# berkeley-hipie/HIPIE

Measured on AMD Instinct MI355X. Metric: images/sec @1024x1024 ViT-H bs=8 (single-image inference hot path: box, class and mask logits), higher is better.
Workload: dtype f16x3 (split-fp16 operands, fp32 accumulate: fp32-class); 1 GPU; BASELINE.json configs[2]: vit_huge, 1024x1024, batch 8 per GPU, 80 class prompts (L=194), detection; global_batch=8, parallelism=dp1, precision_policy=split, launch=eager

## Files before the change

hipie_amd/csrc/gemm.hip:

```cpp
#include "gemm_tile.h"

namespace hipie {

template <typename T>
__global__ __launch_bounds__(256) void to_hl8_kernel(const T* __restrict__ x, f16_t* __restrict__ out, long rows, int K, long ldx, long ldo,
                                                     float scale) {
  const long gid = (long)blockIdx.x * 256 + threadIdx.x;
  const int gpr = K / 8;
  if (gid >= rows * gpr) return;
  const long r = gid / gpr;
  const int g = (int)(gid - r * gpr);
  const T* src = x + r * ldx + 8 * g;
  f16x8 h, l;
#pragma unroll
  for (int e = 0; e < 8; ++e) {
    f16_t hh, ll;
    hl_split((float)src[e] * scale, hh, ll);
    h[e] = hh;
    l[e] = ll;
  }
  f16_t* dst = out + r * ldo + 16 * g;
  *reinterpret_cast<f16x8*>(dst) = h;
  *reinterpret_cast<f16x8*>(dst + 8) = l;
}


constexpr int kTrRows = 128, kTrCols = 64;
__global__ __launch_bounds__(256) void to_hl8_t_kernel(const float* __restrict__ x, f16_t* __restrict__ out, long rows, int C, long ldx,
                                                       long ldo, long rows_p, float scale) {
  __shared__ float tile[kTrRows][kTrCols + 1];
  const long r0 = (long)blockIdx.x * kTrRows;
  const int c0 = blockIdx.y * kTrCols;
  const int tid = threadIdx.x;
  for (int k = tid; k < kTrRows * (kTrCols / 4); k += 256) {
    const int i = k / (kTrCols / 4), j = (k % (kTrCols / 4)) * 4;
    float v[4] = {0.f, 0.f, 0.f, 0.f};
    if (r0 + i < rows) {
      const float* src = x + (r0 + i) * ldx + c0 + j;
      if (c0 + j + 3 < C && (((uintptr_t)src) & 15) == 0) {
        const float4 q = *reinterpret_cast<const float4*>(src);
        v[0] = q.x; v[1] = q.y; v[2] = q.z; v[3] = q.w;
      } else {
        for (int e = 0; e < 4; ++e) v[e] = c0 + j + e < C ? src[e] : 0.f;
      }
    }
    for (int e = 0; e < 4; ++e) tile[i][j + e] = v[e];
  }
  __syncthreads();
  for (int u = tid; u < kTrCols * (kTrRows / 8); u += 256) {
    const int g = u % (kTrRows / 8), c = u / (kTrRows / 8);
    const long m = r0 + 8 * g;
    if (c0 + c >= C || m >= rows_p) continue;
    f16x8 h, l;
#pragma unroll
    for (int e = 0; e < 8; ++e) {
      f16_t hh, ll;
      hl_split(tile[8 * g + e][c] * scale, hh, ll);
      h[e] = hh;
      l[e] = ll;
    }
    f16_t* dst = out + (long)(c0 + c) * ldo + 2 * m;
    *reinterpret_cast<f16x8*>(dst) = h;
    *reinterpret_cast<f16x8*>(dst + 8) = l;
  }
}

}

using namespace hipie;

namespace hipie {
int launch_gemm_k256(const void* X, long ldx_b, int x_f32, const void* W, long ldw_b, const float* bias, float* out, long ldo, int M, int N,
                     hipStream_t st);
}

static inline bool gemm_mfma16() {
  const char* e = study_env("HIPIE_GEMM_MFMA");
  return e ? atoi(e) == 16 : true;
}

static int gemm_impl(const void* A, int64_t lda, const void* W, int64_t ldw, const float* bias, const float* resid, int64_t ldr,
                     void* out, int64_t ldo, const int32_t* out_row, const int32_t* a_row, int64_t a_rows, int M, int N, int K, int in_fmt,
                     int out_fmt, int act, float alpha, float oscale, void* stream, const float* alpha_dev = nullptr) {
  HIPIE_REQUIRE(A && W && out, "gemm: null pointer");
  HIPIE_REQUIRE(in_fmt == HIPIE_F16 || in_fmt == HIPIE_HL8 || in_fmt == HIPIE_F32, "gemm: operand format %d (HIPIE_F16 | HIPIE_HL8 | HIPIE_F32)",
                in_fmt);
  HIPIE_REQUIRE(out_fmt == HIPIE_F32 || out_fmt == HIPIE_F16 || out_fmt == HIPIE_HL8, "gemm: output format %d", out_fmt);
  HIPIE_REQUIRE(act >= 0 && act <= 3, "gemm: activation %d (0 none, 1 gelu, 2 relu, 3 quick-gelu)", act);
  HIPIE_REQUIRE(M > 0 && N > 0 && K > 0 && N % 8 == 0, "gemm: M=%d N=%d K=%d (N must be a multiple of 8)", M, N, K);
  const bool a_f32 = in_fmt == HIPIE_F32;
  const bool split = in_fmt == HIPIE_HL8 || a_f32;
  if (a_f32) lda *= 2;
  const int kq = split ? 32 : 64;
  HIPIE_REQUIRE(K % kq == 0, "gemm: K=%d must be a multiple of %d", K, kq);
  const int epr = split ? 2 * K : K;
  HIPIE_TRY(gm_check_operands("gemm", lda, ldw, epr, 320));
  HIPIE_TRY(gm_check_out("gemm", ldo, out_fmt, N));
  HIPIE_TRY(gm_check_resid("gemm", resid, ldr, N));
  HIPIE_TRY(gm_check_aligned("gemm", {A, W, out, bias, resid}));
  GemmParams p;
  gm_set_operands(p, A, lda, W, ldw, M, N, K, kq);
  p.bias = bias; p.resid = resid; p.ldr = ldr; p.out = (char*)out; p.ldo = ldo; p.out_row = out_row; p.a_row = a_row;
  p.out_fmt = out_fmt; p.act = act; p.alpha = alpha; p.oscale = oscale; p.alpha_dev = alpha_dev;
  hipStream_t st = (hipStream_t)stream;
  static const int k256_mode = [] { const char* e = study_env("HIPIE_GEMM_K256"); return e ? atoi(e) : 2; }();
  const bool k256_on = k256_mode == 1 || (k256_mode == 2 && N >= 384);
  if (k256_on && split && K == 256 && out_fmt == HIPIE_F32 && act == 0 && resid == nullptr && out_row == nullptr && a_row == nullptr &&
      alpha == 1.f && oscale == 1.f && alpha_dev == nullptr && N % 32 == 0 && M >= 8192 && ldw * 2 == 1024 && (long)M * p.lda_b < (1L << 32))
    return launch_gemm_k256(A, p.lda_b, a_f32 ? 1 : 0, W, p.ldw_b, bias, (float*)out, ldo, M, N, st);
  const bool wide = (N % 320 == 0);
  static const int small_on = [] { const char* e = study_env("HIPIE_GEMM_SMALL"); return e ? atoi(e) : 1; }();
  static const long small_tiles = [] { const char* e = study_env("HIPIE_GEMM_SMALL_MAXTILES"); return e ? atol(e) : 96L; }();
  const bool small_ok = small_on && (long)((M + 255) / 256) * ((N + (wide ? 319 : 255)) / (wide ? 320 : 256)) < small_tiles;
#ifdef HIPIE_GEMM_VARIANTS
  { const char* e = study_env("HIPIE_GEMM_VARIANT"); const int v = e ? atoi(e) : 0;
    if (split && wide && v == 1) return launch_gemm<320, true, 1>(p, st);
    if (split && wide && v == 3) return launch_gemm<320, true, 3>(p, st); }
  { const char* e = study_env("HIPIE_GEMM_VARIANT"); if (e) p.variant = atoi(e); }
  p.prio_mode = gemm2_prio();
  if (split && gemm2_mode() == 4) {
    const bool w160 = (N % 160 == 0);
    if (a_f32) return w160 ? launch_gemm4<5, 2>(p, st) : launch_gemm4<4, 2>(p, st);
    return w160 ? launch_gemm4<5, 0>(p, st) : launch_gemm4<4, 0>(p, st);
  }
  if (split && gemm2_mode() == 2) {
    const bool w160 = (N % 160 == 0);
    if (a_f32) return w160 ? launch_gemm3<5, 2>(p, st) : launch_gemm3<4, 2>(p, st);
    return w160 ? launch_gemm3<5, 0>(p, st) : launch_gemm3<4, 0>(p, st);
  }
  if (split && gemm2_mode() == 1) {
    const bool w160 = (N % 160 == 0);
    if (a_f32) return w160 ? launch_gemm2<5, 2>(p, st) : launch_gemm2<4, 2>(p, st);
    return w160 ? launch_gemm2<5, 0>(p, st) : launch_gemm2<4, 0>(p, st);
  }
#endif
  if (split && small_ok && a_row == nullptr) return a_f32 ? launch_gemm_small<2>(p, st) : launch_gemm_small<0>(p, st);
  if (split && wide && gemm_mfma16()) return a_f32 ? launch_gemm<320, true, 2, 16>(p, st) : launch_gemm<320, true, 0, 16>(p, st);
  if (a_f32) return wide ? launch_gemm<320, true, 2>(p, st) : launch_gemm<256, true, 2>(p, st);
  if (split) return wide ? launch_gemm<320, true>(p, st) : launch_gemm<256, true>(p, st);
  return wide ? launch_gemm<320, false>(p, st) : launch_gemm<256, false>(p, st);
}

extern "C" int hipie_gemm(const void* A, int64_t lda, const void* W, int64_t ldw, const float* bias, const float* resid, int64_t ldr,
                          void* out, int64_t ldo, const int32_t* out_row, int M, int N, int K, int in_fmt, int out_fmt, int act, float alpha,
                          float oscale, void* stream) {
  return gemm_impl(A, lda, W, ldw, bias, resid, ldr, out, ldo, out_row, nullptr, 0, M, N, K, in_fmt, out_fmt, act, alpha, oscale, stream);
}

extern "C" int hipie_gemm_scaled(const void* A, int64_t lda, const void* W, int64_t ldw, const float* bias, const float* resid, int64_t ldr,
                                 void* out, int64_t ldo, const int32_t* out_row, int M, int N, int K, int in_fmt, int out_fmt, int act, float alpha,
                                 float oscale, const float* alpha_dev, void* stream) {
  HIPIE_REQUIRE(((uintptr_t)alpha_dev % 4) == 0, "gemm_scaled: alpha_dev must be 4-byte aligned");
  return gemm_impl(A, lda, W, ldw, bias, resid, ldr, out, ldo, out_row, nullptr, 0, M, N, K, in_fmt, out_fmt, act, alpha, oscale, stream, alpha_dev);
}

extern "C" int hipie_gemm_gather(const void* A, int64_t lda, int64_t a_rows, const int32_t* a_row, const void* W, int64_t ldw, const float* bias,
                                 const float* resid, int64_t ldr, void* out, int64_t ldo, const int32_t* out_row, int M, int N, int K, int in_fmt,
                                 int out_fmt, int act, float alpha, float oscale, void* stream) {
  HIPIE_REQUIRE(a_row != nullptr && a_rows > 0, "gemm_gather: a_row map / operand row count missing");
  HIPIE_REQUIRE(in_fmt == HIPIE_HL8 || in_fmt == HIPIE_F32, "gemm_gather: split operands only (HIPIE_HL8 | HIPIE_F32 rows)");
  HIPIE_REQUIRE((long)a_rows * lda * (in_fmt == HIPIE_F32 ? 4 : 2) < (1L << 32), "gemm_gather: the gathered operand must stay below 4 GiB");
  return gemm_impl(A, lda, W, ldw, bias, resid, ldr, out, ldo, out_row, a_row, a_rows, M, N, K, in_fmt, out_fmt, act, alpha, oscale, stream);
}

extern "C" int hipie_gemm_batched(const void* A, int64_t lda, int64_t a_outer, int64_t a_inner, const void* W, int64_t ldw, int64_t w_outer,
                                  int64_t w_inner, void* out, int64_t ldo, int64_t o_outer, int64_t o_inner, int n_outer, int n_inner, int M,
                                  int N, int K, int out_fmt, float alpha, void* stream) {
  HIPIE_REQUIRE(A && W && out, "gemm_batched: null pointer");
  HIPIE_REQUIRE(out_fmt == HIPIE_F32 || out_fmt == HIPIE_HL8, "gemm_batched: output format %d (HIPIE_F32 | HIPIE_HL8)", out_fmt);
  HIPIE_REQUIRE(M > 0 && N > 0 && K > 0 && N % 8 == 0 && K % 32 == 0, "gemm_batched: M=%d N=%d K=%d (N %% 8, K %% 32)", M, N, K);
  HIPIE_TRY(gm_check_batch_shape("gemm_batched", n_outer, n_inner));
  HIPIE_TRY(gm_check_operands("gemm_batched", lda, ldw, 2 * K, 320));
  HIPIE_TRY(gm_check_out("gemm_batched", ldo, out_fmt, N));
  HIPIE_TRY(gm_check_batch_offsets("gemm_batched", a_outer, a_inner, w_outer, w_inner, o_outer, o_inner));
  HIPIE_TRY(gm_check_aligned("gemm_batched", {A, W, out}));
  GemmParams p;
  gm_set_operands(p, A, lda, W, ldw, M, N, K);
  gm_set_batch(p, n_inner, a_outer, a_inner, w_outer, w_inner, o_outer, o_inner, out_fmt == HIPIE_F32 ? 4 : 2);
  p.out = (char*)out; p.ldo = ldo; p.out_fmt = out_fmt; p.alpha = alpha;
  hipStream_t st = (hipStream_t)stream;
  const int batches = n_outer * n_inner;
#ifdef HIPIE_GEMM_VARIANTS
  if (gemm2_mode() == 1) return (N % 160 == 0) ? launch_gemm2<5, 0>(p, st, batches) : launch_gemm2<4, 0>(p, st, batches);
#endif
  return (N % 320 == 0) ? launch_gemm<320, true>(p, st, batches) : launch_gemm<256, true>(p, st, batches);
}

extern "C" int hipie_gemm_batched_resid(const void* A, int64_t lda, int64_t a_outer, int64_t a_inner, const void* W, int64_t ldw, int64_t w_outer,
                                        int64_t w_inner, const float* bias, const float* resid, int64_t ldr, int64_t r_outer, int64_t r_inner,
                                        float* out, int64_t ldo, int64_t o_outer, int64_t o_inner, int n_outer, int n_inner, int M, int N, int K,
                                        float alpha, void* stream) {
  HIPIE_REQUIRE(A && W && out, "gemm_batched_resid: null pointer");
  HIPIE_REQUIRE(M > 0 && N > 0 && K > 0 && N % 8 == 0 && K % 32 == 0, "gemm_batched_resid: M=%d N=%d K=%d (N %% 8, K %% 32)", M, N, K);
  HIPIE_TRY(gm_check_batch_shape("gemm_batched_resid", n_outer, n_inner));
  HIPIE_TRY(gm_check_operands("gemm_batched_resid", lda, ldw, 2 * K, 320));
  HIPIE_TRY(gm_check_out("gemm_batched_resid", ldo, HIPIE_F32, N));
  HIPIE_REQUIRE(resid == nullptr || (ldr >= N && ldr % 4 == 0 && ((r_outer | r_inner) % 4) == 0), "gemm_batched_resid: residual strides %ld / %ld / %ld",
                (long)ldr, (long)r_outer, (long)r_inner);
  HIPIE_TRY(gm_check_batch_offsets("gemm_batched_resid", a_outer, a_inner, w_outer, w_inner, o_outer, o_inner));
  HIPIE_TRY(gm_check_aligned("gemm_batched_resid", {A, W, out, bias, resid}));
  GemmParams p;
  gm_set_operands(p, A, lda, W, ldw, M, N, K);
  gm_set_batch(p, n_inner, a_outer, a_inner, w_outer, w_inner, o_outer, o_inner, 4);
  p.out = (char*)out; p.ldo = ldo; p.alpha = alpha;
  p.bias = bias; p.resid = resid; p.ldr = ldr; p.r_bo = r_outer; p.r_bi = r_inner;
  return (N % 320 == 0) ? launch_gemm<320, true>(p, (hipStream_t)stream, n_outer * n_inner) : launch_gemm<256, true>(p, (hipStream_t)stream, n_outer * n_inner);
}

extern "C" int hipie_gemm_batched_softmax(const void* A, int64_t lda, int64_t a_outer, int64_t a_inner, const void* W, int64_t ldw, int64_t w_outer,
                                          int64_t w_inner, void* out, int64_t ldo, int64_t o_outer, int64_t o_inner, int n_outer, int n_inner,
                                          int M, int N, int K, const unsigned char* mask, int L, float clamp, float alpha, void* stream) {
  HIPIE_REQUIRE(A && W && out, "gemm_batched_softmax: null pointer");
  HIPIE_REQUIRE(M > 0 && N > 0 && N <= 256 && N % 8 == 0 && K > 0 && K % 32 == 0 && L > 0 && L <= N,
                "gemm_batched_softmax: M=%d N=%d K=%d L=%d (N <= 256: the row must fit one column tile)", M, N, K, L);
  HIPIE_TRY(gm_check_batch_shape("gemm_batched_softmax", n_outer, n_inner));
  HIPIE_TRY(gm_check_operands("gemm_batched_softmax", lda, ldw, 2 * K, 320));
  HIPIE_TRY(gm_check_out("gemm_batched_softmax", ldo, HIPIE_HL8, N));
  HIPIE_TRY(gm_check_batch_offsets("gemm_batched_softmax", a_outer, a_inner, w_outer, w_inner, o_outer, o_inner));
  HIPIE_TRY(gm_check_aligned("gemm_batched_softmax", {A, W, out}));
  GemmParams p;
  gm_set_operands(p, A, lda, W, ldw, M, N, K);
  gm_set_batch(p, n_inner, a_outer, a_inner, w_outer, w_inner, o_outer, o_inner, 2);
  p.out = (char*)out; p.ldo = ldo; p.out_fmt = HIPIE_HL8; p.alpha = alpha;
  p.softmax = 1; p.sm_L = L; p.sm_clamp = clamp; p.sm_mask = mask;
  return launch_gemm<256, true>(p, (hipStream_t)stream, n_outer * n_inner);
}

extern "C" int hipie_conv3x3_split(const void* x, int64_t ldx, const void* w, const float* bias, void* out, int64_t ldo, int64_t rows, int Wp,
                                   int C, int N, int in_fmt, int out_fmt, int act, void* stream) {
  HIPIE_REQUIRE(x && w && out, "conv3x3_split: null pointer");
  HIPIE_REQUIRE(in_fmt == HIPIE_HL8 || in_fmt == HIPIE_F32, "conv3x3_split: input format %d (HIPIE_HL8 | HIPIE_F32 rows)", in_fmt);
  HIPIE_REQUIRE(out_fmt == HIPIE_F32 || out_fmt == HIPIE_HL8, "conv3x3_split: output format %d (HIPIE_F32 | HIPIE_HL8)", out_fmt);
  HIPIE_REQUIRE(act >= 0 && act <= 2, "conv3x3_split: activation %d", act);
  HIPIE_REQUIRE(rows > 0 && rows < (1L << 31) && Wp >= 3 && C > 0 && C % 32 == 0 && N > 0 && N % 8 == 0, "conv3x3_split: rows=%ld Wp=%d C=%d N=%d",
                (long)rows, Wp, C, N);
  if (in_fmt == HIPIE_F32) ldx *= 2;
  HIPIE_REQUIRE(ldx >= 2 * C && ldx % 8 == 0, "conv3x3_split: input row stride %ld", (long)ldx);
  HIPIE_REQUIRE((long)(256 + Wp + 2) * ldx * 2 < (1L << 31), "conv3x3_split: row stride too large");
  HIPIE_TRY(gm_check_out("conv3x3_split", ldo, out_fmt, N));
  HIPIE_TRY(gm_check_aligned("conv3x3_split", {x, w, out, bias}));
  GemmParams p;
  gm_set_operands(p, x, ldx, w, (long)2 * 9 * C, (int)rows, N, 9 * C);
  p.bias = bias; p.out = (char*)out; p.ldo = ldo; p.out_fmt = out_fmt; p.act = act;
  p.conv_kpt = C / 32; p.conv_wp = Wp;
  hipStream_t st = (hipStream_t)stream;
  const bool wide = (N % 320 == 0);
  if (in_fmt == HIPIE_F32) return wide ? launch_gemm<320, true, 2>(p, st) : launch_gemm<256, true, 2>(p, st);
  return wide ? launch_gemm<320, true>(p, st) : launch_gemm<256, true>(p, st);
}

extern "C" int hipie_to_hl8(const void* x, int64_t ldx, void* out, int64_t ldo, int64_t rows, int K, int x_dtype, float scale, void* stream) {
  HIPIE_REQUIRE(x && out && rows > 0 && K > 0 && K % 8 == 0, "to_hl8: rows=%ld K=%d (K must be a multiple of 8)", (long)rows, K);
  HIPIE_REQUIRE(ldx >= K && ldo >= 2 * K && ldo % 8 == 0, "to_hl8: row strides %ld / %ld", (long)ldx, (long)ldo);
  const long n = rows * (K / 8);
  const dim3 grid((unsigned)((n + 255) / 256));
  hipStream_t st = (hipStream_t)stream;
  switch (x_dtype) {
    case HIPIE_F32: hipLaunchKernelGGL(to_hl8_kernel<float>, grid, dim3(256), 0, st, (const float*)x, (f16_t*)out, rows, K, ldx, ldo, scale); break;
    case HIPIE_F16: hipLaunchKernelGGL(to_hl8_kernel<f16_t>, grid, dim3(256), 0, st, (const f16_t*)x, (f16_t*)out, rows, K, ldx, ldo, scale); break;
    default: return set_err(HIPIE_EINVAL, "to_hl8: dtype %d", x_dtype);
  }
  return check_launch("to_hl8");
}

extern "C" int hipie_to_hl8_t(const void* x, int64_t ldx, void* out, int64_t ldo, int64_t rows, int C, int64_t rows_p, float scale, void* stream) {
  HIPIE_REQUIRE(x && out && rows > 0 && C > 0, "to_hl8_t: rows=%ld C=%d", (long)rows, C);
  HIPIE_REQUIRE(rows_p >= rows && rows_p % 8 == 0 && ldx >= C && ldo >= 2 * rows_p && ldo % 8 == 0, "to_hl8_t: rows_p=%ld (>= rows, multiple of 8), strides %ld / %ld",
                (long)rows_p, (long)ldx, (long)ldo);
  HIPIE_REQUIRE(((uintptr_t)out % 16) == 0, "to_hl8_t: output must be 16-byte aligned");
  const long tiles_r = (rows_p + kTrRows - 1) / kTrRows, tiles_c = (C + kTrCols - 1) / kTrCols;
  HIPIE_REQUIRE(tiles_c <= 65535, "to_hl8_t: C=%d too wide", C);
  hipLaunchKernelGGL(to_hl8_t_kernel, dim3((unsigned)tiles_r, (unsigned)tiles_c), dim3(256), 0, (hipStream_t)stream, (const float*)x, (f16_t*)out,
                     (long)rows, C, (long)ldx, (long)ldo, (long)rows_p, scale);
  return check_launch("to_hl8_t");
}
```

hipie_amd/csrc/layernorm.hip:

```cpp
#include "common.h"
#include "row_norm.h"

namespace hipie {

struct hl8_t { unsigned int u; };
template <> struct Vec4<hl8_t> {
  static __device__ __forceinline__ void load(const hl8_t* p, float (&v)[4]) {
    const char* q = reinterpret_cast<const char*>(p);
    const bool second = (reinterpret_cast<uintptr_t>(q) & 16) != 0;
    const f16x4 h = *reinterpret_cast<const f16x4*>(second ? q - 8 : q);
    const f16x4 l = *reinterpret_cast<const f16x4*>(second ? q + 8 : q + 16);
#pragma unroll
    for (int i = 0; i < 4; ++i) v[i] = (float)h[i] + (float)l[i];
  }
  static __device__ __forceinline__ void store(hl8_t* p, const float (&v)[4]) {
    char* q = reinterpret_cast<char*>(p);
    const bool second = (reinterpret_cast<uintptr_t>(q) & 16) != 0;
    f16x4 h, l;
#pragma unroll
    for (int i = 0; i < 4; ++i) {
      f16_t hh, ll;
      hl_split(v[i], hh, ll);
      h[i] = hh;
      l[i] = ll;
    }
    *reinterpret_cast<f16x4*>(second ? q - 8 : q) = h;
    *reinterpret_cast<f16x4*>(second ? q + 8 : q + 16) = l;
  }
};

template <typename Tx, typename Td, typename Tn>
__global__ __launch_bounds__(256) void add_layernorm_kernel(const Tx* __restrict__ x, const Td* __restrict__ delta,
                                                            const float* __restrict__ gamma, const float* __restrict__ beta,
                                                            Tx* __restrict__ res_out, Tn* __restrict__ norm_out, long rows,
                                                            int C, float eps, const int32_t* __restrict__ delta_row,
                                                            const int32_t* __restrict__ out_src, const Tn* __restrict__ addend,
                                                            Tn* __restrict__ sum_out) {
  const long orow = (long)blockIdx.x * 4 + (threadIdx.x >> 6);
  if (orow >= rows) return;
  const LnRow r(C);
  const long row = out_src ? (long)out_src[orow] : orow;
  if (row < 0) {
    const float z[4] = {0.f, 0.f, 0.f, 0.f};
    for (int i = 0; i <= r.nv; ++i)
      if ((i < r.nv)|| (r.lane < r.tail)) Vec4<Tn>::store(norm_out + orow * C + r.col(i), z);
    return;
  }
  const long drow = delta_row ? (long)delta_row[row] : row;
  float v[LN_MAXV][4];
  float sum = 0.f;
  const Tx* xr = x + row * C;
#pragma unroll
  for (int i = 0; i < LN_MAXV; ++i) {
    if (r.on(i)) {
      const int c = r.col(i);
      Vec4<Tx>::load(xr + c, v[i]);
      if (delta != nullptr) {
        float d[4];
        Vec4<Td>::load(delta + drow * C + c, d);
#pragma unroll
        for (int e = 0; e < 4; ++e) v[i][e] += d[e];
      }
      if (res_out != nullptr) Vec4<Tx>::store(res_out + row * C + c, v[i]);
#pragma unroll
      for (int e = 0; e < 4; ++e) sum += v[i][e];
    } else {
#pragma unroll
      for (int e = 0; e < 4; ++e) v[i][e] = 0.f;
    }
  }
  sum = wave_sum(sum);
  const float mean = sum / (float)C;
  float sq = 0.f;
#pragma unroll
  for (int i = 0; i < LN_MAXV; ++i) {
    if (r.on(i)) {
#pragma unroll
      for (int e = 0; e < 4; ++e) { const float d = v[i][e] - mean; sq += d * d; }
    }
  }
  sq = wave_sum(sq);
  const float rstd = rsqrtf(sq / (float)C + eps);
#pragma unroll
  for (int i = 0; i < LN_MAXV; ++i) {
    if (r.on(i)) {
      const int c = r.col(i);
      float o[4];
      ln_affine(v[i], mean, rstd, gamma + c, beta + c, o);
      Vec4<Tn>::store(norm_out + orow * C + c, o);
      if (sum_out != nullptr) {
        float a[4];
        Vec4<Tn>::load(addend + orow * C + c, a);
#pragma unroll
        for (int e = 0; e < 4; ++e) a[e] += o[e];
        Vec4<Tn>::store(sum_out + orow * C + c, a);
      }
    }
  }
}

struct LnArgs {
  const void* x; const void* delta; const float* gamma; const float* beta; void* res_out; void* norm_out;
  long rows; int C; float eps;
  int x_dtype, delta_dtype, norm_dtype;
  hipStream_t stream;
  const int32_t* delta_row = nullptr; const int32_t* out_src = nullptr;
  const void* addend = nullptr; void* sum_out = nullptr;
};

template <typename Tx, typename Td, typename Tn>
static int launch_ln(const LnArgs& a) {
  hipLaunchKernelGGL((add_layernorm_kernel<Tx, Td, Tn>), dim3((unsigned)((a.rows + 3) / 4)), dim3(256), 0, a.stream, (const Tx*)a.x,
                     (const Td*)a.delta, a.gamma, a.beta, (Tx*)a.res_out, (Tn*)a.norm_out, a.rows, a.C, a.eps, a.delta_row, a.out_src,
                     (const Tn*)a.addend, (Tn*)a.sum_out);
  return check_launch("add_layernorm");
}

static int add_layernorm(const LnArgs& a) {
  HIPIE_REQUIRE(a.x && a.gamma && a.beta && a.norm_out, "add_layernorm: null pointer");
  HIPIE_REQUIRE(a.rows >= 0 && a.C > 0 && a.C % 4 == 0 && a.C <= LN_MAXV * 256, "add_layernorm: C=%d must be a multiple of 4 and <= %d", a.C, LN_MAXV * 256);
  if (a.rows == 0) return HIPIE_OK;
  return with_dtype(a.x_dtype, "add_layernorm: bad x dtype", [&](auto tx) {
    return with_dtype(a.delta_dtype, "add_layernorm: bad delta dtype", [&](auto td) {
      using Tx = decltype(tx);
      using Td = decltype(td);
      if (a.norm_dtype == HIPIE_HL8) {
        if (a.C % 8 != 0 || (reinterpret_cast<uintptr_t>(a.norm_out) & 31) != 0) return set_err(HIPIE_EINVAL, "add_layernorm: HL8 output needs C %% 8 == 0 and a 32-byte aligned buffer");
        return launch_ln<Tx, Td, hl8_t>(a);
      }
      return with_dtype(a.norm_dtype, "add_layernorm: bad norm dtype", [&](auto tn) { return launch_ln<Tx, Td, decltype(tn)>(a); });
    });
  });
}


template <typename Td, typename Ta>
__global__ __launch_bounds__(256) void add_layernorm_dec_kernel(const float* __restrict__ x, const Td* __restrict__ delta,
                                                                const float* __restrict__ gamma, const float* __restrict__ beta,
                                                                float* __restrict__ norm_out, Ta* __restrict__ norm16,
                                                                const Ta* __restrict__ addend, Ta* __restrict__ sum16, long rows,
                                                                int C, float eps) {
  const long row = (long)blockIdx.x * 4 + (threadIdx.x >> 6);
  if (row >= rows) return;
  const LnRow r(C);
  float v[LN_MAXV][4];
  float sum = 0.f;
#pragma unroll
  for (int i = 0; i < LN_MAXV; ++i) {
    if (r.on(i)) {
      const long c = row * C + r.col(i);
      float d[4];
      Vec4<float>::load(x + c, v[i]);
      Vec4<Td>::load(delta + c, d);
#pragma unroll
      for (int e = 0; e < 4; ++e) { v[i][e] += d[e]; sum += v[i][e]; }
    } else {
#pragma unroll
      for (int e = 0; e < 4; ++e) v[i][e] = 0.f;
    }
  }
  float mean, rstd;
  ln_row_stats(r, v, sum, C, eps, mean, rstd);
#pragma unroll
  for (int i = 0; i < LN_MAXV; ++i) {
    if (r.on(i)) {
      const int cc = r.col(i);
      const long c = row * C + cc;
      float o[4];
      ln_affine(v[i], mean, rstd, gamma + cc, beta + cc, o);
      Vec4<float>::store(norm_out + c, o);
      if (norm16 != nullptr) Vec4<Ta>::store(norm16 + c, o);
      if (sum16 != nullptr) {
        float a[4];
        Vec4<Ta>::load(addend + c, a);
#pragma unroll
        for (int e = 0; e < 4; ++e) a[e] += o[e];
        Vec4<Ta>::store(sum16 + c, a);
      }
    }
  }
}

template <typename Td, typename Ta>
static int launch_ln_dec(const float* x, const void* d, const float* g, const float* b, float* n, void* n16, const void* add,
                         void* s16, long rows, int C, float eps, hipStream_t st) {
  hipLaunchKernelGGL((add_layernorm_dec_kernel<Td, Ta>), dim3((unsigned)((rows + 3) / 4)), dim3(256), 0, st, x, (const Td*)d, g, b,
                     n, (Ta*)n16, (const Ta*)add, (Ta*)s16, rows, C, eps);
  return check_launch("add_layernorm_dec");
}

template <typename Ta>
__global__ __launch_bounds__(256) void add_cast_kernel(const float* __restrict__ a, const Ta* __restrict__ b, Ta* __restrict__ out, long n4) {
  const long i = (long)blockIdx.x * 256 + threadIdx.x;
  if (i >= n4) return;
  float x[4], y[4];
  Vec4<float>::load(a + 4 * i, x);
  Vec4<Ta>::load(b + 4 * i, y);
#pragma unroll
  for (int e = 0; e < 4; ++e) x[e] += y[e];
  Vec4<Ta>::store(out + 4 * i, x);
}

}

extern "C" int hipie_add_layernorm(const void* x, const void* delta, const float* gamma, const float* beta, void* res_out,
                                   void* norm_out, int64_t rows, int C, float eps, int x_dtype, int delta_dtype,
                                   int norm_dtype, void* stream) {
  return hipie::add_layernorm({x, delta, gamma, beta, res_out, norm_out, rows, C, eps, x_dtype, delta_dtype, norm_dtype, (hipStream_t)stream});
}

extern "C" int hipie_add_layernorm_rows(const void* x, const void* delta, const float* gamma, const float* beta,
                                        void* res_out, void* norm_out, int64_t out_rows, int C, float eps, int x_dtype,
                                        int delta_dtype, int norm_dtype, const int32_t* delta_row, const int32_t* out_src,
                                        void* stream) {
  hipie::LnArgs a = {x, delta, gamma, beta, res_out, norm_out, out_rows, C, eps, x_dtype, delta_dtype, norm_dtype, (hipStream_t)stream};
  a.delta_row = delta_row;
  a.out_src = out_src;
  return hipie::add_layernorm(a);
}

extern "C" int hipie_add_layernorm_dec(const float* x, const void* delta, const float* gamma, const float* beta, float* norm_out,
                                       void* norm16_out, const void* addend, void* sum16_out, int64_t rows, int C, float eps,
                                       int delta_dtype, int aux_dtype, void* stream) {
  using namespace hipie;
  HIPIE_REQUIRE(x && delta && gamma && beta && norm_out, "add_layernorm_dec: null pointer");
  HIPIE_REQUIRE((sum16_out == nullptr) || (addend != nullptr), "add_layernorm_dec: sum16_out needs addend");
  HIPIE_REQUIRE(rows >= 0 && C > 0 && C % 4 == 0 && C <= LN_MAXV * 256, "add_layernorm_dec: C=%d must be a multiple of 4 and <= %d", C, LN_MAXV * 256);
  HIPIE_REQUIRE(aux_dtype == HIPIE_F16 || aux_dtype == HIPIE_BF16 || aux_dtype == HIPIE_HL8, "add_layernorm_dec: aux dtype must be f16, bf16 or HL8");
  HIPIE_REQUIRE(aux_dtype != HIPIE_HL8 || (C % 8 == 0 && (((uintptr_t)norm16_out | (uintptr_t)addend | (uintptr_t)sum16_out) & 31) == 0),
                "add_layernorm_dec: HL8 outputs need C %% 8 == 0 and 32-byte aligned buffers");
  if (rows == 0) return HIPIE_OK;
  hipStream_t st = (hipStream_t)stream;
  return with_dtype(delta_dtype, "add_layernorm_dec: bad delta dtype", [&](auto td) {
    auto launch = [&](auto ta) {
      return launch_ln_dec<decltype(td), decltype(ta)>(x, delta, gamma, beta, norm_out, norm16_out, addend, sum16_out, rows, C, eps, st);
    };
    return aux_dtype == HIPIE_F16 ? launch(f16_t()) : aux_dtype == HIPIE_HL8 ? launch(hl8_t()) : launch(bf16_t());
  });
}

extern "C" int hipie_add_cast(const float* a, const void* b, void* out, int64_t n, int dtype, void* stream) {
  using namespace hipie;
  HIPIE_REQUIRE(a && b && out, "add_cast: null pointer");
  HIPIE_REQUIRE(n >= 0 && n % 4 == 0, "add_cast: n must be a multiple of 4");
  HIPIE_REQUIRE(dtype == HIPIE_F16 || dtype == HIPIE_BF16 || dtype == HIPIE_HL8, "add_cast: dtype must be f16, bf16 or HL8");
  HIPIE_REQUIRE(dtype != HIPIE_HL8 || (n % 8 == 0 && (((uintptr_t)b | (uintptr_t)out) & 31) == 0), "add_cast: HL8 needs n %% 8 == 0 and 32-byte aligned buffers");
  if (n == 0) return HIPIE_OK;
  hipStream_t st = (hipStream_t)stream;
  const long n4 = n / 4;
  const unsigned grid = (unsigned)((n4 + 255) / 256);
  auto launch = [&](auto t) {
    using Ta = decltype(t);
    hipLaunchKernelGGL((add_cast_kernel<Ta>), dim3(grid), dim3(256), 0, st, a, (const Ta*)b, (Ta*)out, n4);
  };
  if (dtype == HIPIE_HL8) launch(hl8_t());
  else if (dtype == HIPIE_F16) launch(f16_t());
  else launch(bf16_t());
  return check_launch("add_cast");
}

extern "C" int hipie_add_layernorm_sum(const void* x, const void* delta, const float* gamma, const float* beta, void* res_out,
                                       void* norm_out, const void* addend, void* sum_out, int64_t rows, int C, float eps,
                                       int x_dtype, int delta_dtype, int norm_dtype, void* stream) {
  using namespace hipie;
  HIPIE_REQUIRE((addend == nullptr) == (sum_out == nullptr), "add_layernorm_sum: addend and sum_out go together");
  LnArgs a = {x, delta, gamma, beta, res_out, norm_out, rows, C, eps, x_dtype, delta_dtype, norm_dtype, (hipStream_t)stream};
  a.addend = addend;
  a.sum_out = sum_out;
  return add_layernorm(a);
}
```

hipie_amd/modeling/vit.py:

```python
import math

import torch
import torch.nn as nn
import torch.nn.functional as F

from .. import ops
from ..derived import derived, stamp


def get_rel_pos(q_size, k_size, rel_pos):
    max_rel_dist = int(2 * max(q_size, k_size) - 1)
    if rel_pos.shape[0] != max_rel_dist:
        r = F.interpolate(rel_pos.reshape(1, rel_pos.shape[0], -1).permute(0, 2, 1), size=max_rel_dist, mode="linear")
        r = r.reshape(-1, max_rel_dist).permute(1, 0)
    else:
        r = rel_pos
    q_coords = torch.arange(q_size, device=rel_pos.device)[:, None] * max(k_size / q_size, 1.0)
    k_coords = torch.arange(k_size, device=rel_pos.device)[None, :] * max(q_size / k_size, 1.0)
    rel = (q_coords - k_coords) + (k_size - 1) * max(q_size / k_size, 1.0)
    return r[rel.long()]


def resize_rel_pos(size, rel_pos):
    n = 2 * size - 1
    if rel_pos.shape[0] == n:
        return rel_pos
    r = F.interpolate(rel_pos.reshape(1, rel_pos.shape[0], -1).permute(0, 2, 1), size=n, mode="linear")
    return r.reshape(-1, n).permute(1, 0)


def get_abs_pos(abs_pos, has_cls_token, hw):
    h, w = hw
    if has_cls_token:
        abs_pos = abs_pos[:, 1:]
    size = int(math.sqrt(abs_pos.shape[1]))
    if size != h or size != w:
        new = F.interpolate(abs_pos.reshape(1, size, size, -1).permute(0, 3, 1, 2), size=(h, w), mode="bicubic",
                            align_corners=False)
        return new.permute(0, 2, 3, 1)
    return abs_pos.reshape(1, h, w, -1)


def window_partition(x, ws):
    B, H, W, C = x.shape
    ph, pw = (ws - H % ws) % ws, (ws - W % ws) % ws
    if ph or pw:
        x = F.pad(x, (0, 0, 0, pw, 0, ph))
    Hp, Wp = H + ph, W + pw
    x = x.view(B, Hp // ws, ws, Wp // ws, ws, C)
    return x.permute(0, 1, 3, 2, 4, 5).contiguous().view(-1, ws, ws, C), (Hp, Wp)


def window_unpartition(win, ws, pad_hw, hw):
    Hp, Wp = pad_hw
    H, W = hw
    B = win.shape[0] // (Hp * Wp // ws // ws)
    x = win.view(B, Hp // ws, Wp // ws, ws, ws, -1).permute(0, 1, 3, 2, 4, 5).contiguous().view(B, Hp, Wp, -1)
    if Hp > H or Wp > W:
        x = x[:, :H, :W, :].contiguous()
    return x


_ROW_MAPS = {}
_PAD_ROWS = {}


def window_pad_rows(out_src):
    key = (out_src.data_ptr(), out_src.numel(), str(out_src.device))
    r = _PAD_ROWS.get(key)
    if r is None:
        r = _PAD_ROWS[key] = torch.nonzero(out_src < 0).flatten().to(torch.int32).contiguous()
    return r


class _QkvBuffers(object):

    def __init__(self):
        import collections
        import os
        self.budget = int(float(os.environ.get("HIPIE_QKV_CACHE_GB", "8")) * (1 << 30))
        self.entries = collections.OrderedDict()
        self.shared = {}

    def _live_bytes(self):
        for k in [k for k, e in self.entries.items() if e[0]() is None]:
            del self.entries[k]
        return sum(e[2] for e in self.entries.values())

    def get(self, owner, rows, width, device, pad_rows, bias_row, bias_ver):
        import weakref
        key = (rows, width, str(device), pad_rows.data_ptr(), pad_rows.numel())
        st = owner.__dict__.get("_qkv_state")
        if st is not None and st[0] == key:
            if id(owner) in self.entries:
                self.entries.move_to_end(id(owner))
            if st[2] != bias_ver:
                ops.fill_rows(st[1], pad_rows, bias_row)
                owner._qkv_state = (key, st[1], bias_ver)
            return st[1]
        owner._qkv_state = None
        self.entries.pop(id(owner), None)
        need = rows * width * 2
        while self._live_bytes() + need > self.budget:
            victim = next((k for k, e in self.entries.items() if e[1] != key), None)
            if victim is None:
                break
            blk = self.entries.pop(victim)[0]()
            if blk is not None:
                blk._qkv_state = None
        if self._live_bytes() + need <= self.budget:
            buf = torch.empty(rows, width, dtype=torch.float16, device=device)
            ops.fill_rows(buf, pad_rows, bias_row)
            owner._qkv_state = (key, buf, bias_ver)
            self.entries[id(owner)] = (weakref.ref(owner), key, need)
            return buf
        buf = self.shared.get(key)
        if buf is None:
            self.shared.clear()
            buf = self.shared[key] = torch.empty(rows, width, dtype=torch.float16, device=device)
        return ops.fill_rows(buf, pad_rows, bias_row)


QKV_BUFFERS = _QkvBuffers()


def window_row_maps(B, H, W, ws, device):
    key = (B, H, W, ws, str(device))
    m = _ROW_MAPS.get(key)
    if m is None:
        assert B * H * W < (1 << 24)
        tok = torch.arange(B * H * W, dtype=torch.float32).view(B, H, W, 1)
        win, _ = window_partition(tok + 1.0, ws)
        out_src = (win.reshape(-1) - 1.0).to(torch.int32)
        valid = out_src >= 0
        delta_row = torch.empty(B * H * W, dtype=torch.int32)
        delta_row[out_src[valid].long()] = torch.nonzero(valid).flatten().to(torch.int32)
        m = (out_src.to(device), delta_row.to(device), win.shape[0])
        _ROW_MAPS[key] = m
    return m


class PatchEmbed(nn.Module):

    def __init__(self, kernel_size=(16, 16), stride=(16, 16), in_chans=3, embed_dim=768):
        super().__init__()
        self.proj = nn.Conv2d(in_chans, embed_dim, kernel_size=kernel_size, stride=stride)
        self.patch = kernel_size[0]

    def forward(self, x):
        B, C, H, W = x.shape
        p = self.patch
        w = self.proj.weight
        x = x.reshape(B, C, H // p, p, W // p, p).permute(0, 2, 4, 1, 3, 5).reshape(B, H // p, W // p, C * p * p)
        if getattr(self, "split", False) and x.is_cuda and ops.split_ok(x.shape[-1]):
            return ops.split_linear(x.contiguous(), self, "proj", w, self.proj.bias, weight_fn=lambda: w.reshape(w.shape[0], -1))
        return F.linear(x.to(w.dtype), w.reshape(w.shape[0], -1), self.proj.bias)


class Attention(nn.Module):

    def __init__(self, dim, num_heads, input_size, precision):
        super().__init__()
        self.num_heads = num_heads
        self.scale = (dim // num_heads) ** -0.5
        self.qkv = nn.Linear(dim, dim * 3, bias=True)
        self.proj = nn.Linear(dim, dim)
        self.rel_pos_h = nn.Parameter(torch.zeros(2 * input_size[0] - 1, dim // num_heads))
        self.rel_pos_w = nn.Parameter(torch.zeros(2 * input_size[1] - 1, dim // num_heads))
        self.precision = precision

    def forward(self, x):
        B, H, W, C = x.shape
        nh = self.num_heads
        hd = C // nh
        if ops.vit_attn_rel_ok((H, W), hd):
            w, b, th, tw = self._folded(H, W)
            qkv16 = F.linear(x.to(w.dtype), w, b).reshape(B, H * W, 3 * C).to(self.precision.attn).contiguous()
            o = ops.vit_attn_rel(qkv16, th, tw, (H, W), nh, fast=self.precision.attn_fast)
        else:
            qkv16 = self.qkv(x).reshape(B, H * W, 3 * C).to(self.precision.attn).contiguous()
            th, tw = self._rel_tables(H, W)
            rel_h, rel_w = ops.vit_relpos(qkv16, th, tw, (H, W), nh)
            o = ops.vit_attn(qkv16, rel_h, rel_w, (H, W), nh, self.scale)
        return self.proj(o.to(x.dtype)).view(B, H, W, C)

    def forward_split(self, y, B, H, W, resid, out_row=None, tok2win=None):
        C = self.qkv.weight.shape[1]
        nh = self.num_heads
        c1 = self.scale * ops.LOG2E

        def wq():
            w = self.qkv.weight.detach().float().clone()
            w[:C] *= c1
            return w

        def bq():
            b = self.qkv.bias.detach().float().clone()
            b[:C] *= c1
            return b
        if getattr(self.precision, "vit_attn16", False) and ops.vit_attn_rel_ok((H, W), C // nh):
            qkv16 = ops.split_linear(y, self, "qkv", self.qkv.weight, self.qkv.bias, out_fmt=ops.F16, x_hl8=True, weight_fn=wq, bias_fn=bq,
                                     tag="gemm_qkv")
            th, tw = derived(self, "tabs16", self._params(), lambda: (
                (resize_rel_pos(H, self.rel_pos_h.float()) / self.scale).half().contiguous(),
                (resize_rel_pos(W, self.rel_pos_w.float()) / self.scale).half().contiguous()), extra=(H, W))
            o16 = ops.vit_attn_rel(qkv16.view(B, H * W, 3 * C), th, tw, (H, W), nh, fast=True)
            o = ops.to_hl8(o16.view(B * H * W, C))
            return ops.split_linear(o, self, "proj", self.proj.weight, self.proj.bias, x_hl8=True, tag="gemm_proj",
                                    resid=resid, out=resid, out_row=out_row)
        if tok2win is not None:
            rows = y.shape[0]
            w_, b_, _ = ops.split_weight(self, "qkv", [self.qkv.weight, self.qkv.bias], wq, bq)
            bias_hl8 = derived(self, "bias_hl8", self._params(), lambda: ops.to_hl8(b_.view(1, -1)).view(-1))
            qkv = QKV_BUFFERS.get(self, rows, 6 * C, y.device, window_pad_rows(out_row), bias_hl8, stamp(self._params()))
            ops.split_linear(y, self, "qkv", self.qkv.weight, self.qkv.bias, out_fmt=ops.HL8, x_hl8=True, weight_fn=wq, bias_fn=bq,
                             tag="gemm_qkv", out=qkv, out_row=tok2win, a_row=tok2win)
        else:
            qkv = ops.split_linear(y, self, "qkv", self.qkv.weight, self.qkv.bias, out_fmt=ops.HL8, x_hl8=True, weight_fn=wq, bias_fn=bq,
                                   tag="gemm_qkv")
        th, tw = derived(self, "tabs", self._params(), lambda: (
            ops.hl8_pack(resize_rel_pos(H, self.rel_pos_h.float()) / self.scale),
            ops.hl8_pack(resize_rel_pos(W, self.rel_pos_w.float()) / self.scale)), extra=(H, W))
        o = ops.vit_attn_split(qkv.view(B, H * W, 6 * C), th, tw, (H, W), nh)
        if tok2win is not None:
            return ops.split_linear(o.view(B * H * W, 2 * C), self, "proj", self.proj.weight, self.proj.bias, x_hl8=True, tag="gemm_proj",
                                    resid=resid, out=resid, a_row=tok2win)
        return ops.split_linear(o.view(B * H * W, 2 * C), self, "proj", self.proj.weight, self.proj.bias, x_hl8=True, tag="gemm_proj",
                                resid=resid, out=resid, out_row=out_row)

    def _params(self):
        return (self.qkv.weight, self.qkv.bias, self.rel_pos_h, self.rel_pos_w)

    def _folded(self, H, W):
        def build():
            C = self.qkv.weight.shape[1]
            c1 = self.scale * ops.LOG2E
            w = self.qkv.weight.float().clone()
            b = self.qkv.bias.float().clone()
            w[:C] *= c1
            b[:C] *= c1
            gd = self.qkv.weight.dtype
            th = (resize_rel_pos(H, self.rel_pos_h.float()) / self.scale).to(self.precision.attn).contiguous()
            tw = (resize_rel_pos(W, self.rel_pos_w.float()) / self.scale).to(self.precision.attn).contiguous()
            return w.to(gd).contiguous(), b.to(gd).contiguous(), th, tw
        return derived(self, "fold", self._params(), build, extra=(H, W, self.precision.attn))

    def _rel_tables(self, H, W):
        return derived(self, "rel", self._params(), lambda: (
            resize_rel_pos(H, self.rel_pos_h.float()).to(self.precision.attn).contiguous(),
            resize_rel_pos(W, self.rel_pos_w.float()).to(self.precision.attn).contiguous()), extra=(H, W, self.precision.attn))


class Mlp(nn.Module):

    def __init__(self, in_features, hidden_features):
        super().__init__()
        self.fc1 = nn.Linear(in_features, hidden_features)
        self.act = nn.GELU()
        self.fc2 = nn.Linear(hidden_features, in_features)

    def forward(self, x):
        return self.fc2(self.act(self.fc1(x)))

    def forward_split(self, h, resid, fp8x=()):
        mid = ops.split_linear(h, self, "fc1", self.fc1.weight, self.fc1.bias, act=ops.ACT_GELU, out_fmt=ops.HL8, x_hl8=True, tag="gemm_fc1")
        if "fc2" in fp8x:
            return ops.f8x_linear(mid, self, "fc2", self.fc2.weight, self.fc2.bias, resid=resid, out=resid)
        return ops.split_linear(mid, self, "fc2", self.fc2.weight, self.fc2.bias, x_hl8=True, tag="gemm_fc2", resid=resid, out=resid)


class Block(nn.Module):

    def __init__(self, dim, num_heads, mlp_ratio, window_size, input_size, precision):
        super().__init__()
        self.norm1 = nn.LayerNorm(dim, eps=1e-6)
        self.attn = Attention(dim, num_heads, input_size if window_size == 0 else (window_size, window_size), precision)
        self.norm2 = nn.LayerNorm(dim, eps=1e-6)
        self.mlp = Mlp(dim, int(dim * mlp_ratio))
        self.window_size = window_size
        self.precision = precision

    def forward(self, x, delta=None):
        gd = self.precision.gemm
        ws = self.window_size
        if self.precision.split and x.is_cuda:
            return self._forward_split(x, delta)
        if ws == 0:
            x, y = ops.add_layernorm(x, delta, self.norm1.weight, self.norm1.bias, self.norm1.eps, gd)
            y = self.attn(y)
            x, h = ops.add_layernorm(x, y.contiguous(), self.norm2.weight, self.norm2.bias, self.norm2.eps, gd)
            return x, self.mlp(h)
        B, H, W, C = x.shape
        out_src, delta_row, nwin = window_row_maps(B, H, W, ws, x.device)
        x, y = ops.add_layernorm(x, delta, self.norm1.weight, self.norm1.bias, self.norm1.eps, gd, out_src=out_src)
        y = self.attn(y.view(nwin, ws, ws, C))
        x, h = ops.add_layernorm(x, y.reshape(-1, C), self.norm2.weight, self.norm2.bias, self.norm2.eps, gd, delta_row=delta_row)
        return x, self.mlp(h)


def _block_forward_split(self, x, delta):
    B, H, W, C = x.shape
    ws = self.window_size
    n1, n2 = self.norm1, self.norm2
    if delta is not None:
        x = x + delta
    xs = x.view(B * H * W, C)
    if ws == 0:
        if not ops.vit_attn_split_ok((H, W), C // self.attn.num_heads):
            raise NotImplementedError("split policy: global attention on a %dx%d token grid (not covered: wider than 96 tokens in BOTH directions)" % (H, W))
        y = ops.add_layernorm(x, None, n1.weight, n1.bias, n1.eps, "hl8")[1]
        self.attn.forward_split(y.view(B * H * W, 2 * C), B, H, W, xs)
    else:
        if not ops.vit_attn_split_ok((ws, ws), C // self.attn.num_heads):
            raise NotImplementedError("split policy: window size %d" % ws)
        out_src, delta_row, nwin = window_row_maps(B, H, W, ws, x.device)
        y = ops.add_layernorm(x, None, n1.weight, n1.bias, n1.eps, "hl8", out_src=out_src)[1]
        trim = not getattr(self.attn.precision, "vit_attn16", False)
        self.attn.forward_split(y, nwin, ws, ws, xs, out_row=out_src, tok2win=delta_row if trim else None)
    h = ops.add_layernorm(x, None, n2.weight, n2.bias, n2.eps, "hl8")[1]
    self.mlp.forward_split(h.view(B * H * W, 2 * C), xs, self.precision.fp8x_linears)
    return x, None


Block._forward_split = _block_forward_split


class ViT(nn.Module):

    def __init__(self, cfg, precision):
        super().__init__()
        E = cfg.vit_embed_dim
        self.patch_embed = PatchEmbed((cfg.vit_patch,) * 2, (cfg.vit_patch,) * 2, 3, E)
        n = (cfg.vit_pretrain_img_size // cfg.vit_patch) ** 2 + 1
        self.pos_embed = nn.Parameter(torch.zeros(1, n, E))
        g = cfg.vit_img_size // cfg.vit_patch
        self.blocks = nn.ModuleList([
            Block(E, cfg.vit_heads, cfg.vit_mlp_ratio, cfg.vit_window if i in cfg.vit_window_blocks else 0, (g, g), precision)
            for i in range(cfg.vit_depth)])
        self.fpn1 = nn.Sequential(nn.ConvTranspose2d(E, E // 2, kernel_size=2, stride=2))
        self.fpn2 = nn.Identity()
        self.fpn3 = nn.MaxPool2d(kernel_size=2, stride=2)
        self.precision = precision
        self._out_feature_channels = {"res3": E // 2, "res4": E, "res5": E}
        self._out_feature_strides = {"res3": 8, "res4": 16, "res5": 32}
        nn.init.trunc_normal_(self.pos_embed, std=0.02)

    size_divisibility = 32

    def forward(self, x):
        gd, ad, rd = self.precision.gemm, self.precision.act, self.precision.resid
        self.patch_embed.split = self.precision.split
        x = self.patch_embed(x).float()
        x = (x + self._abs_pos((x.shape[1], x.shape[2]))).to(rd)
        x, delta = x.contiguous(), None
        for blk in self.blocks:
            x, delta = blk(x, delta)
        x = (x if delta is None else x + delta.to(x.dtype)).to(ad)
        B, H, W, E = x.shape
        wt = self.fpn1[0].weight
        b4 = self.fpn1[0].bias.to(wt.dtype).repeat_interleave(4)
        if self.precision.split and x.is_cuda and ops.split_ok(E) and (E // 2) % 8 == 0:
            res3 = ops.convt2x2_split(x.reshape(B * H * W, E), self, "fpn1", wt, self.fpn1[0].bias, B, H, W).to(ad).permute(0, 3, 1, 2)
        else:
            y = F.linear(x.to(wt.dtype), wt.reshape(E, -1).t(), b4).view(B, H, W, E // 2, 2, 2)
            res3 = y.permute(0, 1, 4, 2, 5, 3).reshape(B, 2 * H, 2 * W, E // 2).to(ad).permute(0, 3, 1, 2)
        xp = x.permute(0, 3, 1, 2)
        return {"res3": res3, "res4": xp, "res5": self.fpn3(xp)}

    def _abs_pos(self, hw):
        return derived(self, "abs_pos", [self.pos_embed], lambda: get_abs_pos(self.pos_embed.float(), True, hw), extra=hw)

    def cast_weights(self):
        gd = self.precision.gemm
        for m in self.modules():
            if isinstance(m, (nn.Linear, nn.Conv2d, nn.ConvTranspose2d)):
                m.to(gd)
        return self


class D2ViT(ViT):

    def output_shape(self):
        return {k: dict(channels=self._out_feature_channels[k], stride=self._out_feature_strides[k]) for k in ("res3", "res4", "res5")}
```

Measured before the change: 43.14 images/sec.

## Skip windowed LN gather in trim path; restructure layernorm loads and hl8 stores

In the windowed trim path, norm1 now writes plain token-order rows with no window gather, and the QKV GEMM reads them directly, scattering its output to window rows rather than gathering its input. This drops the padded window-layout LN output and the a_row indirection. The small-GEMM kernel is now excluded when out_row is set. The layernorm kernel is templated on vector count, with a 2-vector variant for C<=512, and issues all x, delta, gamma and beta loads up front to raise memory-level parallelism. The hl8 store uses a DPP lane swap so each lane writes one 16-byte chunk instead of two 8-byte halves.

```diff
diff --git a/hipie_amd/csrc/gemm.hip b/hipie_amd/csrc/gemm.hip
--- a/hipie_amd/csrc/gemm.hip
+++ b/hipie_amd/csrc/gemm.hip
@@ -134,7 +134,7 @@
     return w160 ? launch_gemm2<5, 0>(p, st) : launch_gemm2<4, 0>(p, st);
   }
 #endif
-  if (split && small_ok && a_row == nullptr) return a_f32 ? launch_gemm_small<2>(p, st) : launch_gemm_small<0>(p, st);
+  if (split && small_ok && a_row == nullptr && out_row == nullptr) return a_f32 ? launch_gemm_small<2>(p, st) : launch_gemm_small<0>(p, st);
   if (split && wide && gemm_mfma16()) return a_f32 ? launch_gemm<320, true, 2, 16>(p, st) : launch_gemm<320, true, 0, 16>(p, st);
   if (a_f32) return wide ? launch_gemm<320, true, 2>(p, st) : launch_gemm<256, true, 2>(p, st);
   if (split) return wide ? launch_gemm<320, true>(p, st) : launch_gemm<256, true>(p, st);
diff --git a/hipie_amd/csrc/layernorm.hip b/hipie_amd/csrc/layernorm.hip
--- a/hipie_amd/csrc/layernorm.hip
+++ b/hipie_amd/csrc/layernorm.hip
@@ -29,7 +29,31 @@
   }
 };
 
-template <typename Tx, typename Td, typename Tn>
+template <typename Tn>
+__device__ __forceinline__ void ln_store(Tn* p, const float (&v)[4]) { Vec4<Tn>::store(p, v); }
+template <>
+__device__ __forceinline__ void ln_store<hl8_t>(hl8_t* p, const float (&v)[4]) {
+  typedef unsigned int u32x2 __attribute__((ext_vector_type(2)));
+  typedef unsigned int u32x4 __attribute__((ext_vector_type(4)));
+  f16x4 h, l;
+#pragma unroll
+  for (int i = 0; i < 4; ++i) {
+    f16_t hh, ll;
+    hl_split(v[i], hh, ll);
+    h[i] = hh;
+    l[i] = ll;
+  }
+  const u32x2 hb = __builtin_bit_cast(u32x2, h), lb = __builtin_bit_cast(u32x2, l);
+  const bool odd = (threadIdx.x & 1) != 0;
+  const u32x2 send = odd ? hb : lb;
+  u32x2 recv;
+#pragma unroll
+  for (int k = 0; k < 2; ++k) recv[k] = (unsigned int)__builtin_amdgcn_update_dpp(0, (int)send[k], 0xB1, 0xF, 0xF, false);
+  const u32x4 out = odd ? u32x4{recv[0], recv[1], lb[0], lb[1]} : u32x4{hb[0], hb[1], recv[0], recv[1]};
+  *reinterpret_cast<u32x4*>(p) = out;
+}
+
+template <typename Tx, typename Td, typename Tn, int NV>
 __global__ __launch_bounds__(256) void add_layernorm_kernel(const Tx* __restrict__ x, const Td* __restrict__ delta,
                                                             const float* __restrict__ gamma, const float* __restrict__ beta,
                                                             Tx* __restrict__ res_out, Tn* __restrict__ norm_out, long rows,
@@ -43,37 +67,53 @@
   if (row < 0) {
     const float z[4] = {0.f, 0.f, 0.f, 0.f};
     for (int i = 0; i <= r.nv; ++i)
-      if ((i < r.nv)|| (r.lane < r.tail)) Vec4<Tn>::store(norm_out + orow * C + r.col(i), z);
+      if ((i < r.nv) || (r.lane < r.tail)) ln_store(norm_out + orow * C + r.col(i), z);
     return;
   }
   const long drow = delta_row ? (long)delta_row[row] : row;
-  float v[LN_MAXV][4];
+  float v[NV][4];
+  const Tx* xr = x + row * C;
+#pragma unroll
+  for (int i = 0; i < NV; ++i)
+    if (i <= r.nv) Vec4<Tx>::load(xr + (r.on(i) ? r.col(i) : 0), v[i]);
+  if (delta != nullptr) {
+    const Td* dr = delta + drow * C;
+    float d[NV][4];
+#pragma unroll
+    for (int i = 0; i < NV; ++i)
+      if (i <= r.nv) Vec4<Td>::load(dr + (r.on(i) ? r.col(i) : 0), d[i]);
+#pragma unroll
+    for (int i = 0; i < NV; ++i)
+#pragma unroll
+      for (int e = 0; e < 4; ++e) v[i][e] += d[i][e];
+  }
+#pragma unroll
+  for (int i = 0; i < NV; ++i)
+#pragma unroll
+    for (int e = 0; e < 4; ++e) v[i][e] = r.on(i) ? v[i][e] : 0.f;
   float sum = 0.f;
-  const Tx* xr = x + row * C;
-#pragma unroll
-  for (int i = 0; i < LN_MAXV; ++i) {
+#pragma unroll
+  for (int i = 0; i < NV; ++i) {
     if (r.on(i)) {
-      const int c = r.col(i);
-      Vec4<Tx>::load(xr + c, v[i]);
-      if (delta != nullptr) {
-        float d[4];
-        Vec4<Td>::load(delta + drow * C + c, d);
-#pragma unroll
-        for (int e = 0; e < 4; ++e) v[i][e] += d[e];
-      }
-      if (res_out != nullptr) Vec4<Tx>::store(res_out + row * C + c, v[i]);
+      if (res_out != nullptr) Vec4<Tx>::store(res_out + row * C + r.col(i), v[i]);
 #pragma unroll
       for (int e = 0; e < 4; ++e) sum += v[i][e];
-    } else {
-#pragma unroll
-      for (int e = 0; e < 4; ++e) v[i][e] = 0.f;
+    }
+  }
+  float gv[NV][4], bv[NV][4];
+#pragma unroll
+  for (int i = 0; i < NV; ++i) {
+    if (i <= r.nv) {
+      const int c = r.on(i) ? r.col(i) : 0;
+      Vec4<float>::load(gamma + c, gv[i]);
+      Vec4<float>::load(beta + c, bv[i]);
     }
   }
   sum = wave_sum(sum);
   const float mean = sum / (float)C;
   float sq = 0.f;
 #pragma unroll
-  for (int i = 0; i < LN_MAXV; ++i) {
+  for (int i = 0; i < NV; ++i) {
     if (r.on(i)) {
 #pragma unroll
       for (int e = 0; e < 4; ++e) { const float d = v[i][e] - mean; sq += d * d; }
@@ -82,17 +122,21 @@
   sq = wave_sum(sq);
   const float rstd = rsqrtf(sq / (float)C + eps);
 #pragma unroll
-  for (int i = 0; i < LN_MAXV; ++i) {
-    if (r.on(i)) {
-      const int c = r.col(i);
-      float o[4];
-      ln_affine(v[i], mean, rstd, gamma + c, beta + c, o);
-      Vec4<Tn>::store(norm_out + orow * C + c, o);
-      if (sum_out != nullptr) {
+  for (int i = 0; i < NV; ++i)
+#pragma unroll
+    for (int e = 0; e < 4; ++e) v[i][e] = (v[i][e] - mean) * rstd * gv[i][e] + bv[i][e];
+#pragma unroll
+  for (int i = 0; i < NV; ++i)
+    if (r.on(i)) ln_store(norm_out + orow * C + r.col(i), v[i]);
+  if (sum_out != nullptr) {
+#pragma unroll
+    for (int i = 0; i < NV; ++i) {
+      if (r.on(i)) {
+        const int c = r.col(i);
         float a[4];
         Vec4<Tn>::load(addend + orow * C + c, a);
 #pragma unroll
-        for (int e = 0; e < 4; ++e) a[e] += o[e];
+        for (int e = 0; e < 4; ++e) a[e] += v[i][e];
         Vec4<Tn>::store(sum_out + orow * C + c, a);
       }
     }
@@ -110,9 +154,10 @@
 
 template <typename Tx, typename Td, typename Tn>
 static int launch_ln(const LnArgs& a) {
-  hipLaunchKernelGGL((add_layernorm_kernel<Tx, Td, Tn>), dim3((unsigned)((a.rows + 3) / 4)), dim3(256), 0, a.stream, (const Tx*)a.x,
-                     (const Td*)a.delta, a.gamma, a.beta, (Tx*)a.res_out, (Tn*)a.norm_out, a.rows, a.C, a.eps, a.delta_row, a.out_src,
-                     (const Tn*)a.addend, (Tn*)a.sum_out);
+  const dim3 grid((unsigned)((a.rows + 3) / 4));
+  auto kern = a.C <= 2 * 256 ? add_layernorm_kernel<Tx, Td, Tn, 2> : add_layernorm_kernel<Tx, Td, Tn, LN_MAXV>;
+  hipLaunchKernelGGL(kern, grid, dim3(256), 0, a.stream, (const Tx*)a.x, (const Td*)a.delta, a.gamma, a.beta, (Tx*)a.res_out,
+                     (Tn*)a.norm_out, a.rows, a.C, a.eps, a.delta_row, a.out_src, (const Tn*)a.addend, (Tn*)a.sum_out);
   return check_launch("add_layernorm");
 }
 
diff --git a/hipie_amd/modeling/vit.py b/hipie_amd/modeling/vit.py
--- a/hipie_amd/modeling/vit.py
+++ b/hipie_amd/modeling/vit.py
@@ -209,12 +209,12 @@
             return ops.split_linear(o, self, "proj", self.proj.weight, self.proj.bias, x_hl8=True, tag="gemm_proj",
                                     resid=resid, out=resid, out_row=out_row)
         if tok2win is not None:
-            rows = y.shape[0]
+            rows = out_row.shape[0]
             w_, b_, _ = ops.split_weight(self, "qkv", [self.qkv.weight, self.qkv.bias], wq, bq)
             bias_hl8 = derived(self, "bias_hl8", self._params(), lambda: ops.to_hl8(b_.view(1, -1)).view(-1))
             qkv = QKV_BUFFERS.get(self, rows, 6 * C, y.device, window_pad_rows(out_row), bias_hl8, stamp(self._params()))
             ops.split_linear(y, self, "qkv", self.qkv.weight, self.qkv.bias, out_fmt=ops.HL8, x_hl8=True, weight_fn=wq, bias_fn=bq,
-                             tag="gemm_qkv", out=qkv, out_row=tok2win, a_row=tok2win)
+                             tag="gemm_qkv", out=qkv, out_row=tok2win)
         else:
             qkv = ops.split_linear(y, self, "qkv", self.qkv.weight, self.qkv.bias, out_fmt=ops.HL8, x_hl8=True, weight_fn=wq, bias_fn=bq,
                                    tag="gemm_qkv")
@@ -314,9 +314,9 @@
         if not ops.vit_attn_split_ok((ws, ws), C // self.attn.num_heads):
             raise NotImplementedError("split policy: window size %d" % ws)
         out_src, delta_row, nwin = window_row_maps(B, H, W, ws, x.device)
-        y = ops.add_layernorm(x, None, n1.weight, n1.bias, n1.eps, "hl8", out_src=out_src)[1]
         trim = not getattr(self.attn.precision, "vit_attn16", False)
-        self.attn.forward_split(y, nwin, ws, ws, xs, out_row=out_src, tok2win=delta_row if trim else None)
+        y = ops.add_layernorm(x, None, n1.weight, n1.bias, n1.eps, "hl8", out_src=None if trim else out_src)[1]
+        self.attn.forward_split(y.view(B * H * W, 2 * C) if trim else y, nwin, ws, ws, xs, out_row=out_src, tok2win=delta_row if trim else None)
     h = ops.add_layernorm(x, None, n2.weight, n2.bias, n2.eps, "hl8")[1]
     self.mlp.forward_split(h.view(B * H * W, 2 * C), xs, self.precision.fp8x_linears)
     return x, None
```

Result: no change. 43.20 images/sec, median of 2 (+0.1%).
